# matthewdm0816/BridgeQA

Measured on AMD Instinct MI355X. Metric: train samples/s (40k-pt scene + 512^2 view, bs16), higher is better.
Workload: dtype bf16

## Files before the change

bridgeqa_amd/csrc/ln.hip:

```cpp
#include <cstdint>
#include <stdlib.h>
#include "bq_common.h"

namespace bq {

typedef __bf16 bf16x4 __attribute__((ext_vector_type(4)));

__device__ __forceinline__ float wave_sum_f32(float v) {
  asm volatile(BQ_DPP_WAVE("v_add_f32_dpp") : "+v"(v));
  return __int_as_float(__builtin_amdgcn_readlane(__float_as_int(v), 63));
}

__device__ __forceinline__ bool ln_keep(unsigned seed, int row, int col, unsigned thresh) {
  unsigned x = seed ^ ((unsigned)row * 0x85EBCA77u) ^ ((unsigned)col * 0xC2B2AE3Du);
  x ^= x >> 16; x *= 0x7feb352du; x ^= x >> 15; x *= 0x846ca68bu; x ^= x >> 16;
  return x >= thresh;
}

struct LnArgs {
  int M, H;
  float eps, inv_keep;
  unsigned thresh, seed;
  const unsigned *seed_ptr;
  unsigned path_thresh;
  float path_inv_keep;
  int rows_per_sample;
  int groups;
  const float *gamma2, *beta2;
  int x_is_sum;
};

__device__ __forceinline__ float ln_path_scale(const LnArgs &a, unsigned seed, int row) {
  if (!a.path_thresh) return 1.0f;
  return ln_keep(seed ^ 0x5bd1e995u, row / a.rows_per_sample, 0x3039, a.path_thresh) ? a.path_inv_keep : 0.0f;
}

__device__ __forceinline__ unsigned ln_seed(const LnArgs &a) {
  return a.seed_ptr ? a.seed_ptr[0] * 2654435761u + a.seed : a.seed;
}

template <int NCH>
__device__ __forceinline__ void load_z(const __bf16 *x, const __bf16 *res, long rowoff, int row, int lane,
                                       const LnArgs &a, unsigned seed, float *z) {
  const float ps = ln_path_scale(a, seed, row);
#pragma unroll
  for (int ch = 0; ch < NCH; ++ch) {
    const int c0 = ch * 256 + lane * 4;
    const bf16x4 xv = *reinterpret_cast<const bf16x4 *>(x + rowoff + c0);
    bf16x4 rv = {(__bf16)0.0f, (__bf16)0.0f, (__bf16)0.0f, (__bf16)0.0f};
    if (res) rv = *reinterpret_cast<const bf16x4 *>(res + rowoff + c0);
#pragma unroll
    for (int j = 0; j < 4; ++j) {
      float v = (float)xv[j];
      if (a.thresh) v = ln_keep(seed, row, c0 + j, a.thresh) ? v * a.inv_keep : 0.0f;
      z[ch * 4 + j] = v * ps + (float)rv[j];
    }
  }
}

template <int NCH>
__global__ __launch_bounds__(256) void drop_add_ln_fwd_kernel(const __bf16 *__restrict__ x,
                                                              const __bf16 *__restrict__ res,
                                                              const float *__restrict__ gamma,
                                                              const float *__restrict__ beta, __bf16 *__restrict__ y,
                                                              __bf16 *__restrict__ sum_out,
                                                              float *__restrict__ mean_out,
                                                              float *__restrict__ rstd_out,
                                                              float *__restrict__ zero_out, LnArgs a) {
  const int lane = threadIdx.x & 63, wid = threadIdx.x >> 6;
  const int grp = blockIdx.y, Mg = a.M / a.groups;
  if (grp) { gamma = a.gamma2; beta = a.beta2; }
  if (zero_out && blockIdx.x == 0)
    for (int c = threadIdx.x; c < 2 * a.H; c += 256) zero_out[grp * 2 * a.H + c] = 0.0f;
  const unsigned seed = ln_seed(a);
  const bf16x4 zero4 = {(__bf16)0.0f, (__bf16)0.0f, (__bf16)0.0f, (__bf16)0.0f};
  bf16x4 cx[NCH], cr[NCH], nx[NCH], nr[NCH];
  auto fetch = [&](int row, bf16x4 (&fx)[NCH], bf16x4 (&fr)[NCH]) {
    const long rowoff = (long)row * a.H;
#pragma unroll
    for (int ch = 0; ch < NCH; ++ch) {
      const int c0 = ch * 256 + lane * 4;
      fx[ch] = *reinterpret_cast<const bf16x4 *>(x + rowoff + c0);
      fr[ch] = res ? *reinterpret_cast<const bf16x4 *>(res + rowoff + c0) : zero4;
    }
  };
  const int row_end = (grp + 1) * Mg, stride = gridDim.x * 4;
  int row0 = grp * Mg + blockIdx.x * 4 + wid;
  if (row0 < row_end) fetch(row0, cx, cr);
  for (int row = row0; row < row_end; row += stride) {
  const bool more = row + stride < row_end;
  if (more) fetch(row + stride, nx, nr);
  const long rowoff = (long)row * a.H;
  float z[4 * NCH];
  {
    const float ps = ln_path_scale(a, seed, row);
#pragma unroll
    for (int ch = 0; ch < NCH; ++ch) {
      const int c0 = ch * 256 + lane * 4;
#pragma unroll
      for (int j = 0; j < 4; ++j) {
        float v = (float)cx[ch][j];
        if (a.thresh) v = ln_keep(seed, row, c0 + j, a.thresh) ? v * a.inv_keep : 0.0f;
        z[ch * 4 + j] = v * ps + (float)cr[ch][j];
      }
    }
  }
  float s = 0.0f;
#pragma unroll
  for (int i = 0; i < 4 * NCH; ++i) s += z[i];
  const float mean = wave_sum_f32(s) / (float)a.H;
  float v = 0.0f;
#pragma unroll
  for (int i = 0; i < 4 * NCH; ++i) { const float d = z[i] - mean; v += d * d; }
  const float rstd = rsqrtf(wave_sum_f32(v) / (float)a.H + a.eps);
#pragma unroll
  for (int ch = 0; ch < NCH; ++ch) {
    const int c0 = ch * 256 + lane * 4;
    const float4 g = *reinterpret_cast<const float4 *>(gamma + c0), bt = *reinterpret_cast<const float4 *>(beta + c0);
    bf16x4 o;
    o[0] = (__bf16)((z[ch * 4 + 0] - mean) * rstd * g.x + bt.x);
    o[1] = (__bf16)((z[ch * 4 + 1] - mean) * rstd * g.y + bt.y);
    o[2] = (__bf16)((z[ch * 4 + 2] - mean) * rstd * g.z + bt.z);
    o[3] = (__bf16)((z[ch * 4 + 3] - mean) * rstd * g.w + bt.w);
    *reinterpret_cast<bf16x4 *>(y + rowoff + c0) = o;
    if (sum_out) {
      bf16x4 zs;
      zs[0] = (__bf16)z[ch * 4 + 0]; zs[1] = (__bf16)z[ch * 4 + 1]; zs[2] = (__bf16)z[ch * 4 + 2]; zs[3] = (__bf16)z[ch * 4 + 3];
      *reinterpret_cast<bf16x4 *>(sum_out + rowoff + c0) = zs;
    }
  }
  if (lane == 0) { mean_out[row] = mean; rstd_out[row] = rstd; }
  if (more) {
#pragma unroll
    for (int ch = 0; ch < NCH; ++ch) { cx[ch] = nx[ch]; cr[ch] = nr[ch]; }
  }
  }
}

template <int NCH>
__global__ __launch_bounds__(256) void drop_add_ln_bwd_kernel(const __bf16 *__restrict__ x,
                                                              const __bf16 *__restrict__ res,
                                                              const float *__restrict__ gamma,
                                                              const __bf16 *__restrict__ dy,
                                                              const __bf16 *__restrict__ dsum,
                                                              const float *__restrict__ mean_in,
                                                              const float *__restrict__ rstd_in,
                                                              __bf16 *__restrict__ dx, __bf16 *__restrict__ dres,
                                                              float *__restrict__ dgb, LnArgs a) {
  constexpr bool DET = false;
#include "ln_bwd_kernel_body.h"
}
template <int NCH>
__global__ __launch_bounds__(256) void drop_add_ln_bwd_kernel_det(const __bf16 *__restrict__ x,
                                                                  const __bf16 *__restrict__ res,
                                                                  const float *__restrict__ gamma,
                                                                  const __bf16 *__restrict__ dy,
                                                                  const __bf16 *__restrict__ dsum,
                                                                  const float *__restrict__ mean_in,
                                                                  const float *__restrict__ rstd_in,
                                                                  __bf16 *__restrict__ dx, __bf16 *__restrict__ dres,
                                                                  float *__restrict__ dgb, LnArgs a) {
  constexpr bool DET = true;
#include "ln_bwd_kernel_body.h"
}

__global__ __launch_bounds__(256) void ln_dgb_fold_det_kernel(const float *__restrict__ slab, float *dgb, int chunks, int N) {
  __shared__ float s[4][64];
  const int cl = threadIdx.x & 63, ph = threadIdx.x >> 6;
  const int c = blockIdx.x * 64 + cl;
  float t[8];
#pragma unroll
  for (int u = 0; u < 8; ++u) t[u] = 0.f;
  if (c < N) {
    int y = ph;
    for (; y + 28 < chunks; y += 32) {
#pragma unroll
      for (int u = 0; u < 8; ++u) t[u] += slab[(long)(y + 4 * u) * N + c];
    }
    for (; y < chunks; y += 4) t[0] += slab[(long)y * N + c];
  }
  s[ph][cl] = ((t[0] + t[1]) + (t[2] + t[3])) + ((t[4] + t[5]) + (t[6] + t[7]));
  __syncthreads();
  if (ph == 0 && c < N) dgb[c] = dgb[c] + ((s[0][cl] + s[1][cl]) + (s[2][cl] + s[3][cl]));
}

typedef __bf16 bf16x8 __attribute__((ext_vector_type(8)));

template <int VEC>
__global__ __launch_bounds__(256) void colsum_kernel(const __bf16 *__restrict__ g, float *__restrict__ out,
                                                     float *partial, unsigned *counter, int M, int N,
                                                     int rows_per_chunk) {
  constexpr int LANES = 256 / VEC, PH = 256 / LANES;
  typedef __bf16 vec_t __attribute__((ext_vector_type(VEC)));
  __shared__ float s[PH][256];
  __shared__ int last;
  const int cg = threadIdx.x % LANES, ph = threadIdx.x / LANES;
  const int c0 = blockIdx.x * 256 + cg * VEC;
  const int r0 = blockIdx.y * rows_per_chunk, r1 = min(M, r0 + rows_per_chunk);
  float acc[VEC];
#pragma unroll
  for (int i = 0; i < VEC; ++i) acc[i] = 0.f;
  if (c0 < N) {
    const __bf16 *p = g + (long)(r0 + ph) * N + c0;
    const long step = (long)PH * N;
    int r = r0 + ph;
    for (; r + 3 * PH < r1; r += 4 * PH, p += 4 * step) {
      const vec_t v0 = *reinterpret_cast<const vec_t *>(p), v1 = *reinterpret_cast<const vec_t *>(p + step),
                  v2 = *reinterpret_cast<const vec_t *>(p + 2 * step), v3 = *reinterpret_cast<const vec_t *>(p + 3 * step);
#pragma unroll
      for (int i = 0; i < VEC; ++i) acc[i] += ((float)v0[i] + (float)v1[i]) + ((float)v2[i] + (float)v3[i]);
    }
    for (; r < r1; r += PH, p += step) {
      const vec_t v = *reinterpret_cast<const vec_t *>(p);
#pragma unroll
      for (int i = 0; i < VEC; ++i) acc[i] += (float)v[i];
    }
  }
#pragma unroll
  for (int i = 0; i < VEC; ++i) s[ph][cg * VEC + i] = acc[i];
  __syncthreads();
  const int c = blockIdx.x * 256 + threadIdx.x;
  float v = 0.f;
#pragma unroll
  for (int q = 0; q < PH; ++q) v += s[q][threadIdx.x];
  if (gridDim.y == 1) {
    if (c < N) out[c] = v;
    return;
  }
  if (c < N) partial[(long)blockIdx.y * N + c] = v;
  if (!counter) return;
  __threadfence();
  __syncthreads();
  if (threadIdx.x == 0) last = atomicAdd(counter + blockIdx.x, 1u) == gridDim.y - 1;
  __syncthreads();
  if (!last) return;
  __threadfence();
  if (c < N) {
    float t = 0.f;
    for (int y = 0; y < (int)gridDim.y; ++y) t += __builtin_nontemporal_load(partial + (long)y * N + c);
    out[c] = t;
  }
  if (threadIdx.x == 0) counter[blockIdx.x] = 0u;
}

template <int VEC>
__global__ __launch_bounds__(1024) void colsum_tall_kernel(const __bf16 *__restrict__ g, float *__restrict__ out, int M,
                                                           int N) {
  constexpr int LANES = 256 / VEC, PH = 1024 / LANES;
  typedef __bf16 vec_t __attribute__((ext_vector_type(VEC)));
  __shared__ float s[PH][256 + 1];
  const int cg = threadIdx.x % LANES, ph = threadIdx.x / LANES;
  const int c0 = blockIdx.x * 256 + cg * VEC;
  float acc[VEC];
#pragma unroll
  for (int i = 0; i < VEC; ++i) acc[i] = 0.f;
  if (c0 < N) {
    const __bf16 *p = g + (long)ph * N + c0;
    const long step = (long)PH * N;
    int r = ph;
    for (; r + 3 * PH < M; r += 4 * PH, p += 4 * step) {
      const vec_t v0 = *reinterpret_cast<const vec_t *>(p), v1 = *reinterpret_cast<const vec_t *>(p + step),
                  v2 = *reinterpret_cast<const vec_t *>(p + 2 * step), v3 = *reinterpret_cast<const vec_t *>(p + 3 * step);
#pragma unroll
      for (int i = 0; i < VEC; ++i) acc[i] += ((float)v0[i] + (float)v1[i]) + ((float)v2[i] + (float)v3[i]);
    }
    for (; r < M; r += PH, p += step) {
      const vec_t v = *reinterpret_cast<const vec_t *>(p);
#pragma unroll
      for (int i = 0; i < VEC; ++i) acc[i] += (float)v[i];
    }
  }
#pragma unroll
  for (int i = 0; i < VEC; ++i) s[ph][cg * VEC + i] = acc[i];
  __syncthreads();
  if (threadIdx.x < 256) {
    const int c = blockIdx.x * 256 + threadIdx.x;
    float t0 = 0.f, t1 = 0.f, t2 = 0.f, t3 = 0.f;
#pragma unroll
    for (int q = 0; q < PH; q += 4) {
      t0 += s[q][threadIdx.x]; t1 += s[q + 1][threadIdx.x]; t2 += s[q + 2][threadIdx.x]; t3 += s[q + 3][threadIdx.x];
    }
    if (c < N) out[c] = (t0 + t1) + (t2 + t3);
  }
}

__global__ __launch_bounds__(256) void colsum_fold_kernel(const float *__restrict__ partial, float *__restrict__ out,
                                                          int chunks, int N) {
  __shared__ float s[4][64];
  const int cl = threadIdx.x & 63, ph = threadIdx.x >> 6;
  const int c = blockIdx.x * 64 + cl;
  float t[8];
#pragma unroll
  for (int u = 0; u < 8; ++u) t[u] = 0.f;
  if (c < N) {
    int y = ph;
    for (; y + 28 < chunks; y += 32) {
#pragma unroll
      for (int u = 0; u < 8; ++u) t[u] += partial[(long)(y + 4 * u) * N + c];
    }
    for (; y < chunks; y += 4) t[0] += partial[(long)y * N + c];
  }
  s[ph][cl] = ((t[0] + t[1]) + (t[2] + t[3])) + ((t[4] + t[5]) + (t[6] + t[7]));
  __syncthreads();
  if (ph == 0 && c < N) out[c] = (s[0][cl] + s[1][cl]) + (s[2][cl] + s[3][cl]);
}

__global__ __launch_bounds__(256) void gelu_fwd_kernel(const __bf16 *__restrict__ x, __bf16 *__restrict__ y, long n8) {
  const long stride = (long)gridDim.x * 256;
  for (long i = (long)blockIdx.x * 256 + threadIdx.x; i < n8; i += stride) {
    const bf16x8 v = *reinterpret_cast<const bf16x8 *>(x + i * 8);
    bf16x8 o;
#pragma unroll
    for (int j = 0; j < 8; ++j) {
      const float f = (float)v[j];
      o[j] = (__bf16)(0.5f * f * (1.0f + erff(f * 0.70710678118654752440f)));
    }
    *reinterpret_cast<bf16x8 *>(y + i * 8) = o;
  }
}

}
using namespace bq;

extern "C" int bq_gelu_fwd_bf16(const void *x, void *y, long n, void *stream) {
  BQ_REQUIRE(n >= 0 && n % 8 == 0, BQ_EINVAL, "gelu: n must be a multiple of 8");
  if (n == 0) return BQ_OK;
  BQ_REQUIRE(x && y && (((uintptr_t)x | (uintptr_t)y) & 15) == 0, BQ_EINVAL, "gelu: null / unaligned pointer");
  const long n8 = n / 8;
  long blocks = (n8 + 255) / 256;
  if (blocks > 4096) blocks = 4096;
  hipLaunchKernelGGL(gelu_fwd_kernel, dim3((unsigned)blocks), dim3(256), 0, (hipStream_t)stream, (const __bf16 *)x,
                     (__bf16 *)y, n8);
  return check_launch("gelu_fwd");
}

#define BQ_COLSUM_ONE_LAUNCH_ROWS 2048
#define BQ_COLSUM_TALL_ROWS 1024
extern "C" int bq_colsum_chunks(int M) {
  if (M <= BQ_COLSUM_TALL_ROWS) return 1;
  const int rpc = M <= BQ_COLSUM_ONE_LAUNCH_ROWS ? 32 : 128;
  return M <= rpc ? 1 : (M + rpc - 1) / rpc;
}

extern "C" int bq_colsum_bf16(const void *g, float *out, int M, int N, float *partial, unsigned *counter, void *stream) {
  BQ_REQUIRE(M >= 0 && N > 0 && N % 4 == 0, BQ_EINVAL, "colsum: bad extents");
  BQ_REQUIRE((g || M == 0) && out, BQ_EINVAL, "colsum: null pointer");
  hipStream_t st = (hipStream_t)stream;
  const int vec = N % 8 == 0 ? 8 : 4;
  if (M <= BQ_COLSUM_TALL_ROWS) {
    const dim3 grid((N + 255) / 256);
    with_int<8, 4>(vec, [&](auto V) {
      hipLaunchKernelGGL(colsum_tall_kernel<decltype(V)::value>, grid, dim3(1024), 0, st, (const __bf16 *)g, out, M, N);
    });
    return check_launch("colsum");
  }
  const int chunks = bq_colsum_chunks(M);
  const bool one_launch = M <= BQ_COLSUM_ONE_LAUNCH_ROWS;
  BQ_REQUIRE(chunks == 1 || (partial && (counter || !one_launch)), BQ_EINVAL, "colsum: workspace missing for %d chunks",
             chunks);
  const int rpc = chunks == 1 ? (M > 0 ? M : 1) : (one_launch ? 32 : 128);
  const dim3 grid((N + 255) / 256, chunks);
  unsigned *cnt = one_launch ? counter : nullptr;
  with_int<8, 4>(vec, [&](auto V) {
    hipLaunchKernelGGL(colsum_kernel<decltype(V)::value>, grid, dim3(256), 0, st, (const __bf16 *)g, out, partial, cnt, M, N, rpc);
  });
  if (chunks > 1 && !one_launch)
    hipLaunchKernelGGL(colsum_fold_kernel, dim3((N + 63) / 64), dim3(256), 0, st, partial, out, chunks, N);
  return check_launch("colsum");
}

static LnArgs ln_args(int M, int H, float eps, float p_drop, float p_path, int rows_per_sample, unsigned seed,
                      const unsigned *seed_ptr, int groups, const float *gamma2, const float *beta2, int x_is_sum) {
  const DropCode drop = drop_code(p_drop), path = drop_code(p_path);
  LnArgs a{};
  a.M = M; a.H = H; a.eps = eps;
  a.inv_keep = drop.inv_keep; a.thresh = drop.thresh;
  a.seed = seed; a.seed_ptr = seed_ptr;
  a.path_thresh = path.thresh; a.path_inv_keep = path.inv_keep; a.rows_per_sample = rows_per_sample;
  a.groups = groups; a.gamma2 = gamma2; a.beta2 = beta2;
  a.x_is_sum = x_is_sum;
  return a;
}

static int ln_fwd_launch(const void *x, const void *residual, const float *gamma, const float *beta, const float *gamma2,
                         const float *beta2, int groups, void *y, void *sum_out, float *mean, float *rstd,
                         float *zero_out, int M, int H, float eps, float p_drop, float p_path, int rows_per_sample,
                         unsigned seed, const unsigned *seed_ptr, void *stream) {
  BQ_REQUIRE(M >= 0 && H > 0 && H % 256 == 0 && H <= 1024, BQ_ELIMIT, "drop_add_ln: H=%d unsupported", H);
  BQ_REQUIRE(groups == 1 || (groups == 2 && gamma2 && beta2 && M % 2 == 0), BQ_EINVAL, "drop_add_ln: bad row groups");
  if (M == 0) {
    if (zero_out) (void)hipMemsetAsync(zero_out, 0, sizeof(float) * 2 * H * groups, (hipStream_t)stream);
    return check_launch("drop_add_ln_fwd");
  }
  BQ_REQUIRE(x && gamma && beta && y && mean && rstd, BQ_EINVAL, "drop_add_ln: null pointer");
  BQ_REQUIRE(p_path == 0.0f || rows_per_sample > 0, BQ_EINVAL, "drop_add_ln: rows_per_sample");
  const LnArgs a = ln_args(M, H, eps, p_drop, p_path, rows_per_sample, seed, seed_ptr, groups, gamma2, beta2, 0);
#ifndef BQ_LN_FWD_CAP
#define BQ_LN_FWD_CAP 1024
#endif
  constexpr int fwd_cap = BQ_LN_FWD_CAP;
  const int Mg = M / groups;
  const dim3 grid(((Mg + 3) / 4) < fwd_cap ? (Mg + 3) / 4 : fwd_cap, groups);
  hipStream_t st = (hipStream_t)stream;
  with_int<1, 2, 3, 4>(H / 256, [&](auto NCH) {
    hipLaunchKernelGGL(drop_add_ln_fwd_kernel<decltype(NCH)::value>, grid, dim3(256), 0, st, (const __bf16 *)x,
                       (const __bf16 *)residual, gamma, beta, (__bf16 *)y, (__bf16 *)sum_out, mean, rstd, zero_out, a);
  });
  return check_launch("drop_add_ln_fwd");
}
extern "C" int bq_drop_add_ln_fwd(
    const void *x, const void *residual, const float *gamma, const float *beta, void *y, void *sum_out, float *mean,
    float *rstd, float *zero_out, int M, int H, float eps, float p_drop, float p_path, int rows_per_sample,
    unsigned seed, const unsigned *seed_ptr, void *stream) {
  return ln_fwd_launch(x, residual, gamma, beta, nullptr, nullptr, 1, y, sum_out, mean, rstd, zero_out, M, H, eps, p_drop,
                       p_path, rows_per_sample, seed, seed_ptr, stream);
}
extern "C" int bq_twin_drop_add_ln_fwd(
    const void *x, const void *residual, const float *gamma, const float *beta, const float *gamma2, const float *beta2,
    void *y, float *mean, float *rstd, float *zero_out, int M, int H, float eps, float p_drop, unsigned seed,
    const unsigned *seed_ptr, void *stream) {
  return ln_fwd_launch(x, residual, gamma, beta, gamma2, beta2, 2, y, nullptr, mean, rstd, zero_out, M, H, eps, p_drop,
                       0.0f, 0, seed, seed_ptr, stream);
}

static int ln_bwd_blocks(int M, int groups) {
  constexpr int bwd_cap = 384;
  const int blocks = (M / groups + 3) / 4;
  return blocks > bwd_cap ? bwd_cap : blocks;
}
static int ln_bwd_launch(const void *x, const void *residual, const float *gamma, const float *gamma2, int groups,
                         const void *dy, const void *dsum, const float *mean, const float *rstd, void *dx,
                         void *dresidual, float *dgb, int M, int H, float eps, float p_drop, float p_path,
                         int rows_per_sample, unsigned seed, const unsigned *seed_ptr, void *stream, int x_is_sum = 0,
                         float *slab = nullptr) {
  BQ_REQUIRE(M >= 0 && H > 0 && H % 256 == 0 && H <= 1024, BQ_ELIMIT, "drop_add_ln: H=%d unsupported", H);
  BQ_REQUIRE(groups == 1 || (groups == 2 && gamma2 && M % 2 == 0), BQ_EINVAL, "drop_add_ln_bwd: bad row groups");
  if (M == 0) return BQ_OK;
  BQ_REQUIRE(x && gamma && dy && mean && rstd && dx && dgb && (x_is_sum ? !residual : (!residual == !dresidual)), BQ_EINVAL,
             "drop_add_ln_bwd: null pointer");
  BQ_REQUIRE(!x_is_sum || (p_drop == 0.0f && groups == 1), BQ_EINVAL, "drop_add_ln_bwd_sum: no dropout, one row group");
  BQ_REQUIRE(p_path == 0.0f || rows_per_sample > 0, BQ_EINVAL, "drop_add_ln_bwd: rows_per_sample");
  const LnArgs a = ln_args(M, H, eps, p_drop, p_path, rows_per_sample, seed, seed_ptr, groups, gamma2, nullptr, x_is_sum);
  const int blocks = ln_bwd_blocks(M, groups);
  hipStream_t st = (hipStream_t)stream;
  auto launch = [&](auto kernel) {
    hipLaunchKernelGGL(kernel, dim3(blocks, groups), dim3(256), 0, st, (const __bf16 *)x, (const __bf16 *)residual, gamma,
                       (const __bf16 *)dy, (const __bf16 *)dsum, mean, rstd, (__bf16 *)dx, (__bf16 *)dresidual,
                       slab ? slab : dgb, a);
  };
  if (slab) {
    with_int<1, 2, 3, 4>(H / 256, [&](auto NCH) { launch(drop_add_ln_bwd_kernel_det<decltype(NCH)::value>); });
    const int N = groups * 2 * H;
    hipLaunchKernelGGL(ln_dgb_fold_det_kernel, dim3((N + 63) / 64), dim3(256), 0, st, (const float *)slab, dgb, blocks, N);
    return check_launch("drop_add_ln_bwd_det");
  }
  with_int<1, 2, 3, 4>(H / 256, [&](auto NCH) { launch(drop_add_ln_bwd_kernel<decltype(NCH)::value>); });
  return check_launch("drop_add_ln_bwd");
}
extern "C" long bq_drop_add_ln_bwd_det_slab_floats(int M, int H, int groups) {
  if (M <= 0 || H <= 0 || groups < 1) return 0;
  return (long)ln_bwd_blocks(M, groups) * groups * 2 * H;
}
extern "C" int bq_drop_add_ln_bwd_det(
    const void *x, const void *residual, const float *gamma, const float *gamma2, int groups, const void *dy, const void *dsum,
    const float *mean, const float *rstd, void *dx, void *dresidual, float *dgb, float *slab, int M, int H, float eps,
    float p_drop, float p_path, int rows_per_sample, unsigned seed, const unsigned *seed_ptr, int x_is_sum, void *stream) {
  BQ_REQUIRE(slab || M == 0, BQ_EINVAL, "drop_add_ln_bwd_det: no slab");
  BQ_REQUIRE(groups == 1 || (!x_is_sum && !dsum && p_path == 0.0f), BQ_EINVAL, "drop_add_ln_bwd_det: two row groups take no sum form");
  return ln_bwd_launch(x, residual, gamma, groups == 2 ? gamma2 : nullptr, groups, dy, dsum, mean, rstd, dx, dresidual, dgb, M, H,
                       eps, p_drop, p_path, rows_per_sample, seed, seed_ptr, stream, x_is_sum ? 1 : 0, slab);
}
extern "C" int bq_drop_add_ln_bwd(
    const void *x, const void *residual, const float *gamma, const void *dy, const void *dsum, const float *mean,
    const float *rstd, void *dx, void *dresidual, float *dgb, int M, int H, float eps, float p_drop, float p_path,
    int rows_per_sample, unsigned seed, const unsigned *seed_ptr, void *stream) {
  return ln_bwd_launch(x, residual, gamma, nullptr, 1, dy, dsum, mean, rstd, dx, dresidual, dgb, M, H, eps, p_drop, p_path,
                       rows_per_sample, seed, seed_ptr, stream);
}
extern "C" int bq_drop_add_ln_bwd_sum(
    const void *sum, const float *gamma, const void *dy, const void *dsum, const float *mean, const float *rstd, void *dx,
    void *dresidual, float *dgb, int M, int H, float eps, float p_path, int rows_per_sample, unsigned seed,
    const unsigned *seed_ptr, void *stream) {
  return ln_bwd_launch(sum, nullptr, gamma, nullptr, 1, dy, dsum, mean, rstd, dx, dresidual, dgb, M, H, eps, 0.0f, p_path,
                       rows_per_sample, seed, seed_ptr, stream, 1);
}
extern "C" int bq_twin_drop_add_ln_bwd(
    const void *x, const void *residual, const float *gamma, const float *gamma2, const void *dy, const float *mean,
    const float *rstd, void *dx, void *dresidual, float *dgb, int M, int H, float eps, float p_drop, unsigned seed,
    const unsigned *seed_ptr, void *stream) {
  return ln_bwd_launch(x, residual, gamma, gamma2, 2, dy, nullptr, mean, rstd, dx, dresidual, dgb, M, H, eps, p_drop, 0.0f,
                       0, seed, seed_ptr, stream);
}
```

bridgeqa_amd/csrc/ln_bwd_kernel_body.h:

```cpp
  __shared__ float s_g[4][256 * NCH], s_b[4][256 * NCH];
  const int lane = threadIdx.x & 63, wid = threadIdx.x >> 6;
  const int grp = blockIdx.y, Mg = a.M / a.groups;
  if constexpr (DET) dgb += (long)blockIdx.x * gridDim.y * 2 * a.H;
  if (grp) { gamma = a.gamma2; dgb += 2 * a.H; }
  const unsigned seed = ln_seed(a);
  float ag[4 * NCH], ab[4 * NCH], gm[4 * NCH];
#pragma unroll
  for (int ch = 0; ch < NCH; ++ch) {
    const float4 g = *reinterpret_cast<const float4 *>(gamma + ch * 256 + lane * 4);
    gm[ch * 4 + 0] = g.x; gm[ch * 4 + 1] = g.y; gm[ch * 4 + 2] = g.z; gm[ch * 4 + 3] = g.w;
  }
#pragma unroll
  for (int i = 0; i < 4 * NCH; ++i) { ag[i] = 0.0f; ab[i] = 0.0f; }
  const float invH = 1.0f / (float)a.H;
  struct Raw {
    bf16x4 x[NCH], r[NCH], d[NCH], s[NCH];
    float mean, rstd;
  };
  const bf16x4 zero4 = {(__bf16)0.0f, (__bf16)0.0f, (__bf16)0.0f, (__bf16)0.0f};
  auto fetch = [&](int row, Raw &w) {
    const long rowoff = (long)row * a.H;
#pragma unroll
    for (int ch = 0; ch < NCH; ++ch) {
      const int c0 = ch * 256 + lane * 4;
      w.x[ch] = *reinterpret_cast<const bf16x4 *>(x + rowoff + c0);
      w.r[ch] = res ? *reinterpret_cast<const bf16x4 *>(res + rowoff + c0) : zero4;
      w.d[ch] = *reinterpret_cast<const bf16x4 *>(dy + rowoff + c0);
      w.s[ch] = dsum ? *reinterpret_cast<const bf16x4 *>(dsum + rowoff + c0) : zero4;
    }
    w.mean = mean_in[row];
    w.rstd = rstd_in[row];
  };
  const int row_end = (grp + 1) * Mg, stride = gridDim.x * 4;
  int row = grp * Mg + blockIdx.x * 4 + wid;
  Raw cur, nxt;
  if (row < row_end) fetch(row, cur);
  for (; row < row_end; row += stride) {
    const bool more = row + stride < row_end;
    if (more) fetch(row + stride, nxt);
    const long rowoff = (long)row * a.H;
    float z[4 * NCH], g[4 * NCH];
    const float ps = ln_path_scale(a, seed, row);
    const float mean = cur.mean, rstd = cur.rstd;
    float s1 = 0.0f, s2 = 0.0f;
#pragma unroll
    for (int ch = 0; ch < NCH; ++ch) {
      const int c0 = ch * 256 + lane * 4;
#pragma unroll
      for (int j = 0; j < 4; ++j) {
        const int i = ch * 4 + j;
        float v = (float)cur.x[ch][j];
        if (a.thresh) v = ln_keep(seed, row, c0 + j, a.thresh) ? v * a.inv_keep : 0.0f;
        z[i] = a.x_is_sum ? v : v * ps + (float)cur.r[ch][j];
        const float dyv = (float)cur.d[ch][j];
        z[i] = (z[i] - mean) * rstd;
        g[i] = dyv * gm[i];
        s1 += g[i];
        s2 += g[i] * z[i];
        ag[i] += dyv * z[i];
        ab[i] += dyv;
      }
    }
    s1 = wave_sum_f32(s1) * invH;
    s2 = wave_sum_f32(s2) * invH;
#pragma unroll
    for (int ch = 0; ch < NCH; ++ch) {
      const int c0 = ch * 256 + lane * 4;
      bf16x4 ox, orr;
#pragma unroll
      for (int j = 0; j < 4; ++j) {
        const int i = ch * 4 + j;
        const float dz = rstd * (g[i] - s1 - z[i] * s2) + (float)cur.s[ch][j];
        orr[j] = (__bf16)dz;
        float dxv = dz * ps;
        if (a.thresh) dxv = ln_keep(seed, row, c0 + j, a.thresh) ? dxv * a.inv_keep : 0.0f;
        ox[j] = (__bf16)dxv;
      }
      *reinterpret_cast<bf16x4 *>(dx + rowoff + c0) = ox;
      if (dres) *reinterpret_cast<bf16x4 *>(dres + rowoff + c0) = orr;
    }
    if (more) cur = nxt;
  }
#pragma unroll
  for (int ch = 0; ch < NCH; ++ch)
#pragma unroll
    for (int j = 0; j < 4; ++j) {
      s_g[wid][ch * 256 + lane * 4 + j] = ag[ch * 4 + j];
      s_b[wid][ch * 256 + lane * 4 + j] = ab[ch * 4 + j];
    }
  __syncthreads();
  constexpr int H = 256 * NCH;
  for (int c = threadIdx.x; c < H; c += 256) {
    if constexpr (DET) {
      dgb[c] = (s_g[0][c] + s_g[1][c]) + (s_g[2][c] + s_g[3][c]);
      dgb[H + c] = (s_b[0][c] + s_b[1][c]) + (s_b[2][c] + s_b[3][c]);
    } else {
      atomicAdd(dgb + c, (s_g[0][c] + s_g[1][c]) + (s_g[2][c] + s_g[3][c]));
      atomicAdd(dgb + H + c, (s_b[0][c] + s_b[1][c]) + (s_b[2][c] + s_b[3][c]));
    }
  }
```

Baseline: 506.6.

## Use wider blocks for long-row LayerNorm backward and drop register prefetch

When a row group has at least 4096 rows, the LayerNorm backward kernel now launches 8-wave blocks with a lower block cap instead of 4-wave blocks. The software double-buffered row prefetch is removed to cut register pressure, relying on more resident waves to hide memory latency. The shared-memory gamma/beta partial reduction now folds waves in groups of four across several barrier passes. The deterministic slab is still sized by the old 4-wave shape, which is at least as large as the new grid needs. The risks are lost latency hiding from the removed prefetch and extra barriers in the reduction.

New measurement: 503.2. Within noise of the previous version (-0.7%).

```diff
diff --git a/bridgeqa_amd/csrc/ln.hip b/bridgeqa_amd/csrc/ln.hip
--- a/bridgeqa_amd/csrc/ln.hip
+++ b/bridgeqa_amd/csrc/ln.hip
@@ -137,8 +137,20 @@
   }
 }
 
+#ifndef BQ_LN_BWD_WAVES
+#define BQ_LN_BWD_WAVES 8
+#endif
+#ifndef BQ_LN_BWD_CAP
+#define BQ_LN_BWD_CAP 256
+#endif
+#ifndef BQ_LN_BWD_LONG_ROWS
+#define BQ_LN_BWD_LONG_ROWS 4096
+#endif
+constexpr int LN_BWD_LONG_WAVES = BQ_LN_BWD_WAVES, LN_BWD_LONG_CAP = BQ_LN_BWD_CAP, LN_BWD_LONG_ROWS = BQ_LN_BWD_LONG_ROWS;
+constexpr int LN_BWD_SHORT_CAP = 384;
+static_assert(LN_BWD_LONG_WAVES % 4 == 0 && LN_BWD_LONG_WAVES <= 16 && LN_BWD_LONG_CAP <= LN_BWD_SHORT_CAP, "ln backward launch shape");
 template <int NCH>
-__global__ __launch_bounds__(256) void drop_add_ln_bwd_kernel(const __bf16 *__restrict__ x,
+__global__ __launch_bounds__(64 * LN_BWD_LONG_WAVES) void drop_add_ln_bwd_kernel(const __bf16 *__restrict__ x,
                                                               const __bf16 *__restrict__ res,
                                                               const float *__restrict__ gamma,
                                                               const __bf16 *__restrict__ dy,
@@ -151,7 +163,7 @@
 #include "ln_bwd_kernel_body.h"
 }
 template <int NCH>
-__global__ __launch_bounds__(256) void drop_add_ln_bwd_kernel_det(const __bf16 *__restrict__ x,
+__global__ __launch_bounds__(64 * LN_BWD_LONG_WAVES) void drop_add_ln_bwd_kernel_det(const __bf16 *__restrict__ x,
                                                                   const __bf16 *__restrict__ res,
                                                                   const float *__restrict__ gamma,
                                                                   const __bf16 *__restrict__ dy,
@@ -423,10 +435,16 @@
                        0.0f, 0, seed, seed_ptr, stream);
 }
 
+static int ln_bwd_waves(int M, int groups) { return M / groups >= LN_BWD_LONG_ROWS ? LN_BWD_LONG_WAVES : 4; }
 static int ln_bwd_blocks(int M, int groups) {
-  constexpr int bwd_cap = 384;
+  const int w = ln_bwd_waves(M, groups);
+  const int bwd_cap = w == 4 ? LN_BWD_SHORT_CAP : LN_BWD_LONG_CAP;
+  const int blocks = (M / groups + w - 1) / w;
+  return blocks > bwd_cap ? bwd_cap : blocks;
+}
+static int ln_bwd_slab_rows(int M, int groups) {
   const int blocks = (M / groups + 3) / 4;
-  return blocks > bwd_cap ? bwd_cap : blocks;
+  return blocks > LN_BWD_SHORT_CAP ? LN_BWD_SHORT_CAP : blocks;
 }
 static int ln_bwd_launch(const void *x, const void *residual, const float *gamma, const float *gamma2, int groups,
                          const void *dy, const void *dsum, const float *mean, const float *rstd, void *dx,
@@ -441,10 +459,10 @@
   BQ_REQUIRE(!x_is_sum || (p_drop == 0.0f && groups == 1), BQ_EINVAL, "drop_add_ln_bwd_sum: no dropout, one row group");
   BQ_REQUIRE(p_path == 0.0f || rows_per_sample > 0, BQ_EINVAL, "drop_add_ln_bwd: rows_per_sample");
   const LnArgs a = ln_args(M, H, eps, p_drop, p_path, rows_per_sample, seed, seed_ptr, groups, gamma2, nullptr, x_is_sum);
-  const int blocks = ln_bwd_blocks(M, groups);
+  const int blocks = ln_bwd_blocks(M, groups), waves = ln_bwd_waves(M, groups);
   hipStream_t st = (hipStream_t)stream;
   auto launch = [&](auto kernel) {
-    hipLaunchKernelGGL(kernel, dim3(blocks, groups), dim3(256), 0, st, (const __bf16 *)x, (const __bf16 *)residual, gamma,
+    hipLaunchKernelGGL(kernel, dim3(blocks, groups), dim3(64 * waves), 0, st, (const __bf16 *)x, (const __bf16 *)residual, gamma,
                        (const __bf16 *)dy, (const __bf16 *)dsum, mean, rstd, (__bf16 *)dx, (__bf16 *)dresidual,
                        slab ? slab : dgb, a);
   };
@@ -459,7 +477,7 @@
 }
 extern "C" long bq_drop_add_ln_bwd_det_slab_floats(int M, int H, int groups) {
   if (M <= 0 || H <= 0 || groups < 1) return 0;
-  return (long)ln_bwd_blocks(M, groups) * groups * 2 * H;
+  return (long)ln_bwd_slab_rows(M, groups) * groups * 2 * H;
 }
 extern "C" int bq_drop_add_ln_bwd_det(
     const void *x, const void *residual, const float *gamma, const float *gamma2, int groups, const void *dy, const void *dsum,
diff --git a/bridgeqa_amd/csrc/ln_bwd_kernel_body.h b/bridgeqa_amd/csrc/ln_bwd_kernel_body.h
--- a/bridgeqa_amd/csrc/ln_bwd_kernel_body.h
+++ b/bridgeqa_amd/csrc/ln_bwd_kernel_body.h
@@ -1,5 +1,5 @@
   __shared__ float s_g[4][256 * NCH], s_b[4][256 * NCH];
-  const int lane = threadIdx.x & 63, wid = threadIdx.x >> 6;
+  const int lane = threadIdx.x & 63, wid = __builtin_amdgcn_readfirstlane(threadIdx.x >> 6), nw = blockDim.x >> 6;
   const int grp = blockIdx.y, Mg = a.M / a.groups;
   if constexpr (DET) dgb += (long)blockIdx.x * gridDim.y * 2 * a.H;
   if (grp) { gamma = a.gamma2; dgb += 2 * a.H; }
@@ -31,13 +31,10 @@
     w.mean = mean_in[row];
     w.rstd = rstd_in[row];
   };
-  const int row_end = (grp + 1) * Mg, stride = gridDim.x * 4;
-  int row = grp * Mg + blockIdx.x * 4 + wid;
-  Raw cur, nxt;
-  if (row < row_end) fetch(row, cur);
-  for (; row < row_end; row += stride) {
-    const bool more = row + stride < row_end;
-    if (more) fetch(row + stride, nxt);
+  const int row_end = (grp + 1) * Mg, stride = gridDim.x * nw;
+  for (int row = grp * Mg + blockIdx.x * nw + wid; row < row_end; row += stride) {
+    Raw cur;
+    fetch(row, cur);
     const long rowoff = (long)row * a.H;
     float z[4 * NCH], g[4 * NCH];
     const float ps = ln_path_scale(a, seed, row);
@@ -79,18 +76,23 @@
       *reinterpret_cast<bf16x4 *>(dx + rowoff + c0) = ox;
       if (dres) *reinterpret_cast<bf16x4 *>(dres + rowoff + c0) = orr;
     }
-    if (more) cur = nxt;
   }
+  for (int w0 = 0; w0 < nw; w0 += 4) {
+    if (wid >= w0 && wid < w0 + 4) {
+      float *ig = s_g[wid & 3], *ib = s_b[wid & 3];
 #pragma unroll
-  for (int ch = 0; ch < NCH; ++ch)
+      for (int ch = 0; ch < NCH; ++ch)
 #pragma unroll
-    for (int j = 0; j < 4; ++j) {
-      s_g[wid][ch * 256 + lane * 4 + j] = ag[ch * 4 + j];
-      s_b[wid][ch * 256 + lane * 4 + j] = ab[ch * 4 + j];
+        for (int j = 0; j < 4; ++j) {
+          const int c = ch * 256 + lane * 4 + j;
+          ig[c] = w0 ? ig[c] + ag[ch * 4 + j] : ag[ch * 4 + j];
+          ib[c] = w0 ? ib[c] + ab[ch * 4 + j] : ab[ch * 4 + j];
+        }
     }
-  __syncthreads();
+    __syncthreads();
+  }
   constexpr int H = 256 * NCH;
-  for (int c = threadIdx.x; c < H; c += 256) {
+  for (int c = threadIdx.x; c < H; c += blockDim.x) {
     if constexpr (DET) {
       dgb[c] = (s_g[0][c] + s_g[1][c]) + (s_g[2][c] + s_g[3][c]);
       dgb[H + c] = (s_b[0][c] + s_b[1][c]) + (s_b[2][c] + s_b[3][c]);
```
